# ibrahimhroob/SPS

Hardware: AMD Instinct MI355X
Metric: scans/sec @100k pts, 0.1 m voxel (higher is better)
Workload: dtype f32; 1 GPU; BASELINE config 2: single ~100k-pt LiDAR-like scan + variant-B submap, 0.1 m voxel, CustomMinkUNet14 fp32, 1 scan per step per GPU (4 distinct scans cycled); scan_points=100824, rows=153557, streams_per_gpu=8, compact_arenas=True

## Files before the change

### include/sps_hip.h

```cpp
#ifndef SPS_HIP_H
#define SPS_HIP_H

#include <stddef.h>
#include <stdint.h>

#ifdef __cplusplus
extern "C" {
#endif

#define SPS_OK 0
#define SPS_ERR_INVALID (-1)
#define SPS_ERR_HIP (-2)
#define SPS_ERR_NOMEM (-3)
#define SPS_ERR_RANGE (-4)
#define SPS_ERR_NOWEIGHTS (-5)
#define SPS_ERR_ITEMCAP (-6)

#define SPS_NUM_LEVELS 5

#define SPS_COORD_MIN (-131072)
#define SPS_COORD_MAX (131071)
#define SPS_T_MIN (-16)
#define SPS_T_MAX (15)
#define SPS_BATCH_MAX (30)
#define SPS_MAX_POINTS (1 << 23)

typedef struct sps_ctx sps_ctx;

const char *sps_last_error(void);
int sps_version(void);

int sps_ctx_create(int device, sps_ctx **out);
int sps_ctx_destroy(sps_ctx *ctx);
int sps_reserve(sps_ctx *ctx, int64_t max_points);
int sps_ctx_set_level_fractions(sps_ctx *ctx, const float *frac);
int64_t sps_arena_bytes(sps_ctx *ctx);
int sps_ctx_set_inference_only(sps_ctx *ctx, int on);
int sps_ctx_set_pipelined(sps_ctx *ctx, int on);

int sps_weights_num_tensors(void);
int sps_weights_tensor_info(int idx, char *name, int name_cap, int64_t *offset, int64_t *numel);
int64_t sps_weights_numel(void);
int sps_weights_load(sps_ctx *ctx, const float *blob_host, int64_t numel);
typedef struct sps_weights_handle sps_weights_handle;
int sps_weights_create(int device, const float *blob_host, int64_t numel, int out_channels, sps_weights_handle **out);
int sps_weights_destroy(sps_weights_handle *w);
int sps_ctx_set_weights(sps_ctx *ctx, sps_weights_handle *w);

int sps_forward(sps_ctx *ctx, const float *coords_dev, int64_t ld, int64_t n, float voxel_size,
                float *scores_dev, void *stream);
int sps_check(sps_ctx *ctx, void *stream);

int sps_forward_metrics(sps_ctx *ctx, const float *batch_dev, int64_t ld, int64_t n, float voxel_size, float eps,
                        int n_batches, float *scores_dev, double *out_dev, void *stream);

int sps_head_num_tensors(int out_channels);
int sps_head_tensor_info(int out_channels, int idx, char *name, int name_cap, int64_t *offset, int64_t *numel);
int64_t sps_head_numel(int out_channels);
int sps_weights_load_head(sps_ctx *ctx, const float *blob_host, int64_t numel, int out_channels);
int sps_forward_head(sps_ctx *ctx, const float *coords_dev, int64_t ld, int64_t n, float voxel_size,
                     const float *feats_dev, float t_base, float *out_dev, int64_t ldo, int activation, void *stream);
// ... 206 lines not shown
```

### sps_amd/_native.py

```python
from __future__ import annotations

import ctypes as C
import os

from . import _build

NUM_LEVELS = 5
SPS_OK = 0
ERR_RANGE = -4
ERR_NOMEM = -3
ERR_INVALID = -1
ERR_ITEMCAP = -6


class SpsError(RuntimeError):
    def __init__(self, code: int, msg: str):
        super().__init__(f"libsps_hip error {code}: {msg}")
        self.code = code


ABI_VERSION = 202


def _load() -> C.CDLL:
    path = os.environ.get("SPS_LIB") or _build.LIB
    if path == _build.LIB and (not os.path.exists(path) or _build.is_stale()):
        if _build.have_hipcc():
            path = _build.build()
        elif not os.path.exists(path):
            raise ImportError("libsps_hip.so is missing and hipcc is not available to build it")
    import importlib.util
    if importlib.util.find_spec("torch") is not None:
        import torch
    lib = C.CDLL(path)
    vp, i64, i32, f32 = C.c_void_p, C.c_int64, C.c_int, C.c_float
    sig = {
        "sps_last_error": (C.c_char_p, []),
        "sps_version": (i32, []),
        "sps_ctx_create": (i32, [i32, C.POINTER(vp)]),
        "sps_ctx_destroy": (i32, [vp]),
        "sps_reserve": (i32, [vp, i64]),
        "sps_ctx_set_level_fractions": (i32, [vp, vp]),
        "sps_ctx_set_inference_only": (i32, [vp, i32]),
        "sps_ctx_set_pipelined": (i32, [vp, i32]),
        "sps_arena_bytes": (i64, [vp]),
        "sps_weights_num_tensors": (i32, []),
        "sps_weights_tensor_info": (i32, [i32, C.c_char_p, i32, C.POINTER(i64), C.POINTER(i64)]),
        "sps_weights_numel": (i64, []),
        "sps_weights_load": (i32, [vp, vp, i64]),
        "sps_weights_create": (i32, [i32, vp, i64, i32, C.POINTER(vp)]),
        "sps_weights_destroy": (i32, [vp]),
        "sps_ctx_set_weights": (i32, [vp, vp]),
        "sps_forward": (i32, [vp, vp, i64, i64, f32, vp, vp]),
        "sps_forward_metrics": (i32, [vp, vp, i64, i64, f32, f32, i32, vp, vp, vp]),
        "sps_head_num_tensors": (i32, [i32]),
        "sps_head_tensor_info": (i32, [i32, i32, C.c_char_p, i32, C.POINTER(i64), C.POINTER(i64)]),
        "sps_head_numel": (i64, [i32]),
        "sps_weights_load_head": (i32, [vp, vp, i64, i32]),
        "sps_forward_head": (i32, [vp, vp, i64, i64, f32, vp, f32, vp, i64, i32, vp]),
        "sps_check": (i32, [vp, vp]),
        "sps_metrics": (i32, [vp, vp, vp, i64, i64, f32, i32, C.POINTER(C.c_double), vp]),
        "sps_metrics_dev": (i32, [vp, vp, vp, i64, i64, f32, i32, vp, vp]),
        "sps_profile_enable": (i32, [vp, i32]),
        "sps_profile_count": (i32, [vp]),
        "sps_profile_read": (i32, [vp, i32, C.c_char_p, i32, C.POINTER(f32)]),
        "sps_profile_kernel": (i32, [vp, i32, C.c_char_p, i32]),
        "sps_map_upload": (i32, [vp, vp, i64, i64, f32, vp]),
# ... 81 lines not shown
        "sps_ndt_source_build": (i32, [vp, vp, vp, i64, C.c_double, i32, C.c_double, vp, vp, vp, vp, vp]),
        "sps_ndt_align_d2d_scratch": (i64, [i64]),
        "sps_ndt_align_d2d": (i32, [vp, vp, vp, i64, vp, i32, i32, i32, C.c_double, C.c_double, C.c_double, vp, vp, vp, vp, vp,
                                    vp]),
        "sps_ukf_state_bytes": (i64, []),
        "sps_ukf_init": (i32, [vp, vp, vp, vp, vp]),
        "sps_ukf_predict": (i32, [vp, vp, i32, vp, vp, vp, vp]),
        "sps_ukf_predict_dt": (i32, [vp, C.c_double, vp, vp, vp, vp]),
        "sps_ukf_correct": (i32, [vp, vp, vp, vp, vp, vp]),
    }
    for name, (res, args) in sig.items():
        fn = getattr(lib, name)
        fn.restype = res
        fn.argtypes = args
    if lib.sps_version() != ABI_VERSION:
        raise ImportError(f"{path} reports ABI version {lib.sps_version()}, this binding needs {ABI_VERSION}: rebuild it "
                          "(python -m sps_amd._build)")
    return lib


lib = _load()
EXPORTS = ["sps_last_error", "sps_version", "sps_ctx_create", "sps_ctx_destroy", "sps_reserve",
           "sps_ctx_set_level_fractions", "sps_ctx_set_inference_only", "sps_ctx_set_pipelined", "sps_arena_bytes",
           "sps_weights_num_tensors", "sps_weights_tensor_info", "sps_weights_numel", "sps_weights_load",
           "sps_weights_create", "sps_weights_destroy", "sps_ctx_set_weights",
           "sps_forward", "sps_forward_metrics", "sps_head_num_tensors", "sps_head_tensor_info", "sps_head_numel", "sps_weights_load_head",
           "sps_forward_head", "sps_check", "sps_metrics", "sps_metrics_dev",
           "sps_profile_enable", "sps_profile_count", "sps_profile_read", "sps_profile_kernel", "sps_map_upload", "sps_map_upload_voxels",
           "sps_submap_voxel", "sps_submap_voxel_ijk", "sps_transform_points", "sps_filter_prepare", "sps_forward_n",
           "sps_compact_stable", "sps_filter_finish", "sps_train_forward", "sps_train_backward", "sps_train_generation", "sps_train_backward_at", "sps_scan_mse", "sps_scan_mse_backward", "sps_radius_grid_upload", "sps_radius_count",
           "sps_radius_fill", "sps_radius_grid_attach", "sps_radius_item", "sps_forward_metrics_n", "sps_level_counts", "sps_get_voxels",
           "sps_get_inverse", "sps_get_parent", "sps_get_map_pairs", "sps_get_tile_masks", "sps_get_nbr", "sps_get_kernel_map", "sps_get_rulebook_chunks", "sps_get_logits", "sps_get_feature",
           "sps_lts_num_tensors", "sps_lts_tensor_info", "sps_lts_numel", "sps_lts_lidar_info", "sps_lts_create",
           "sps_lts_destroy", "sps_lts_project", "sps_lts_forward", "sps_lts_check", "sps_lts_tap",
           "sps_forward_head_n", "sps_transform_rows", "sps_transform_points_n", "sps_radius_crop", "sps_label_filter",
           "sps_loc_downsample_scratch", "sps_loc_align_scratch", "sps_loc_downsample", "sps_loc_align",
           "sps_ndt_align_scratch", "sps_ndt_map_build", "sps_ndt_map_cells", "sps_ndt_align",
           "sps_ndt_align_batch_scratch", "sps_ndt_align_batch",
           "sps_ndt_score_scratch", "sps_ndt_score_poses", "sps_ndt_top_poses",
           "sps_ndt_map_build_dynamic", "sps_ndt_map_update_scratch", "sps_ndt_map_update", "sps_ndt_map_info",
           "sps_ndt_map_carve_scratch", "sps_ndt_map_carve", "sps_ndt_map_carve_cells",
           "sps_ndt_pyramid_build", "sps_ndt_pyramid_cells", "sps_ndt_pyramid_align_scratch", "sps_ndt_pyramid_align",
           "sps_ndt_pyramid_build_dynamic", "sps_ndt_pyramid_update_scratch", "sps_ndt_pyramid_update",
           "sps_ndt_pyramid_carve_scratch", "sps_ndt_pyramid_carve", "sps_ndt_pyramid_info", "sps_ndt_pyramid_carve_cells",
           "sps_ndt_source_scratch", "sps_ndt_source_build", "sps_ndt_align_d2d_scratch", "sps_ndt_align_d2d",
           "sps_ukf_state_bytes", "sps_ukf_init", "sps_ukf_predict", "sps_ukf_predict_dt", "sps_ukf_correct"]
# ... 62 lines not shown
            self.handle = None

    def __del__(self):
        try:
            self.close()
        except Exception:
            pass

    def reserve(self, max_points: int):
        check(lib.sps_reserve(self.handle, int(max_points)))

    LIDAR_FRACTIONS = (1.0, 0.6, 0.3, 0.15, 0.08)

    def set_level_fractions(self, frac=None):
        arr = None if frac is None else (C.c_float * NUM_LEVELS)(*[float(x) for x in frac])
        check(lib.sps_ctx_set_level_fractions(self.handle, arr))

    def set_inference_only(self, on: bool = True):
        check(lib.sps_ctx_set_inference_only(self.handle, 1 if on else 0))

    def set_pipelined(self, on: bool = True):
        check(lib.sps_ctx_set_pipelined(self.handle, 1 if on else 0))

    def arena_bytes(self) -> int:
        return int(lib.sps_arena_bytes(self.handle))

    def load_weights(self, blob_host_ptr: int, numel: int, out_channels: int = 1):
        check(lib.sps_weights_load_head(self.handle, blob_host_ptr, int(numel), int(out_channels)))
        self.weights = None

    def set_weights(self, weights: "Weights"):
        check(lib.sps_ctx_set_weights(self.handle, weights.handle))
        self.weights = weights

    def forward_head(self, coords_ptr: int, ld: int, n: int, voxel_size: float, feats_ptr, t_base: float,
                     out_ptr: int, ldo: int, activation: int, stream: int):
        check(lib.sps_forward_head(self.handle, coords_ptr, ld, n, voxel_size, feats_ptr, t_base, out_ptr, ldo,
                                   activation, stream))

    def forward_head_n(self, coords_ptr: int, ld: int, n_max: int, n_dev_ptr: int, voxel_size: float, feats_ptr,
                       t_base: float, out_ptr: int, ldo: int, activation: int, stream: int):
        check(lib.sps_forward_head_n(self.handle, coords_ptr, ld, n_max, n_dev_ptr, voxel_size, feats_ptr, t_base, out_ptr,
                                     ldo, activation, stream))

    def forward_metrics(self, batch_ptr: int, ld: int, n: int, voxel_size: float, eps: float, n_batches: int,
                        scores_ptr: int, out_ptr: int, stream: int):
# ... 364 lines not shown
```

### sps_amd/csrc/grid_kernels.inc.h

```cpp

typedef unsigned int u32x2 __attribute__((ext_vector_type(2)));
constexpr int SCAN_BLOCK = 1024;

struct BHash {
  uint64_t *keys;
  unsigned long long *mask;
  int *first;
  int *rank;
  uint32_t *occ;
  uint32_t hmask;
  uint32_t hshift;
};

constexpr uint32_t BH_X = 0x9E3779B1u, BH_Y = 0x85EBCA77u, BH_Z = 0xC2B2AE3Du, BH_T = 0x27D4EB2Fu;
__device__ inline uint32_t bhash32(uint64_t key) {
  return (uint32_t)(key & 0x3FFFF) * BH_X + (uint32_t)((key >> 18) & 0x3FFFF) * BH_Y + (uint32_t)((key >> 36) & 0x3FFFF) * BH_Z +
         (uint32_t)(key >> 54) * BH_T;
}

__device__ inline int bhash_insert(const BHash &h, uint64_t key) {
  uint32_t s = bhash32(key) >> h.hshift;
  while (true) {
    unsigned long long prev = atomicCAS(reinterpret_cast<unsigned long long *>(&h.keys[s]),
                                        (unsigned long long)KEY_EMPTY, (unsigned long long)key);
// ... 99 lines not shown
}

struct PyramidArgs {
  BHash h[NLV];
  int *sslot[NLV];
  const unsigned char *sbit0;
  int *bslot[NLV];
  uint64_t *bkey[NLV];
  unsigned long long *bmask[NLV];
  int *bbase[NLV];
  uint4 *bmb[NLV];
  int *bparent[NLV];
  int *bchild[NLV];
  int *badj[NLV];
  int *vblock[NLV];
  unsigned char *vbit[NLV];
  int *counts;
  unsigned long long *agg;
  int agg_stride;
  uint32_t gen;
  const int *n_dev;
  int capl[NLV], bcapl[NLV];
  int *err;
};

constexpr int ABORT = 15;

__device__ inline int block_reduce_sum(int v, int *lds) {
  const int lane = threadIdx.x & 63, wave = threadIdx.x >> 6;
  for (int o = 32; o > 0; o >>= 1) v += __shfl_down(v, o, 64);
  if (lane == 0) lds[wave] = v;
  __syncthreads();
  int tot = 0;
  const int nw = blockDim.x >> 6;
  for (int i = 0; i < nw; ++i) tot += lds[i];
  __syncthreads();
  return tot;
}

constexpr int TICKET = 16, TOCC = 24, N_COUNTERS = 32;

__device__ inline unsigned long long agg_pack(uint32_t gen, int t0, int t1) {
  return ((unsigned long long)gen << 32) | ((unsigned long long)(uint32_t)t1 << 13) | (unsigned long long)(uint32_t)t0;
}
constexpr int SCAN_SPIN_MAX = 1 << 22;
__device__ inline int2 scan_lookback(const unsigned long long *agg, int id, uint32_t gen, int *lds, int *err) {
  if constexpr (SPS_ABLATE_FE & 2) return make_int2(0, 0);
// ... 263 lines not shown
          for (int k = 0; k < 2; ++k)
#pragma unroll
            for (int jj = 0; jj < 2; ++jj)
#pragma unroll
              for (int i = 0; i < 2; ++i)
                if (m & (0x0000000000330033ull << (2 * i + 8 * jj + 32 * k))) {
                  const int bit = (int)((2 * oz + k) * 16 + (2 * oy + jj) * 4 + (2 * ox + i));
                  const int row = base + __popcll(pmask & ((1ull << bit) - 1ull));
                  a.vblock[1][row] = br;
                  a.vbit[1][row] = (unsigned char)bit;
                }
        } else {
          const uint32_t px = (bx >> (j - 2)) & 3, py = (by >> (j - 2)) & 3, pz = (bz >> (j - 2)) & 3;
          const int bit = (int)((pz << 4) | (py << 2) | px);
          const int row = base + __popcll(pmask & ((1ull << bit) - 1ull));
          a.vblock[j][row] = br;
          a.vbit[j][row] = (unsigned char)bit;
        }
      }
    }
  }
}

constexpr int LINK_PER = 3;
#if defined(SPS_FE_TRACE)
__device__ unsigned long long g_link_trace[2 * 16384];
struct LinkStamp {
  __device__ LinkStamp() { if (threadIdx.x == 0 && blockIdx.x < 16384) g_link_trace[2 * blockIdx.x] = wall_clock64(); }
  __device__ ~LinkStamp() { if (threadIdx.x == 0 && blockIdx.x < 16384) g_link_trace[2 * blockIdx.x + 1] = wall_clock64(); }
};
#endif
__global__ __launch_bounds__(256) void k_link_adj(PyramidArgs a, int gb, int c1, int c2, int c3, int c4, int c5) {
  if (a.counts[ABORT]) return;
#if defined(SPS_FE_TRACE)
  LinkStamp stamp;
#endif
  if ((int)blockIdx.x < 4 * gb) {
    link_levels(a, (int)blockIdx.x / gb, (int)blockIdx.x % gb, gb);
    return;
  }
  const int bx = (int)blockIdx.x - 4 * gb;
  const int idx = bx < c1 ? 0 : bx < c2 ? 1 : bx < c3 ? 2 : bx < c4 ? 3 : 4;
  const int level = NLV - 1 - idx;
  const int lo = idx == 0 ? 0 : idx == 1 ? c1 : idx == 2 ? c2 : idx == 3 ? c3 : c4;
  const int hi = idx == 0 ? c1 : idx == 1 ? c2 : idx == 2 ? c3 : idx == 3 ? c4 : c5;
  const int total = a.counts[8 + level] * 27;
  const int lim = 1 << (16 - level);
  const BHash h = a.h[level];
  const uint32_t tocc = reinterpret_cast<const uint32_t *>(a.counts)[TOCC];
  const uint64_t *__restrict__ bkey = a.bkey[level];
  int *__restrict__ badj = a.badj[level];
  const __amdgpu_buffer_rsrc_t rsOcc = __builtin_amdgcn_make_buffer_rsrc((void *)h.occ, 0, (int)0xFFFFFFFEu, 0x00020000);
  const __amdgpu_buffer_rsrc_t rsKeys = __builtin_amdgcn_make_buffer_rsrc((void *)h.keys, 0, (int)0xFFFFFFFEu, 0x00020000);
  const __amdgpu_buffer_rsrc_t rsRank = __builtin_amdgcn_make_buffer_rsrc((void *)h.rank, 0, (int)0xFFFFFFFEu, 0x00020000);
  for (int i = (bx - lo) * 256 + (int)threadIdx.x; i < total; i += (hi - lo) * 256) {
    const int r = i / 27, g = i - r * 27;
    const int dy = g % 3 - 1, dz = (g / 3) % 3 - 1, dt = g / 9 - 1;
    const uint64_t key = bkey[r];
    const int kx = (int)(key & 0x3FFFF), ky = (int)((key >> 18) & 0x3FFFF) + dy, kz = (int)((key >> 36) & 0x3FFFF) + dz,
// ... 76 lines not shown
```

### sps_amd/csrc/sps_hip.hip

```cpp
#include <hip/hip_runtime.h>

#include <cmath>
#include <cstdarg>
#include <cstdint>
#include <cstdio>
#include <algorithm>
#include <array>
#include <cstdlib>
#include <cstring>
#include <map>
#include <memory>
#include <string>
#include <vector>

#include "../../include/sps_hip.h"

#if !defined(SPS_DIAG)
#undef SPS_ABLATE_A
#undef SPS_ABLATE_B
#undef SPS_ABLATE_HALF_B
#undef SPS_ABLATE_SKIP_B
#undef SPS_ABLATE_MFMA
#undef SPS_ABLATE_LOOP
#undef SPS_ABLATE_STAGE
// ... 142 lines not shown
  int device = 0;
  float *blob = nullptr;
  float *ss = nullptr;
  float *wu = nullptr;
  float final_bias = 0.f;
  const NetSpec *net = nullptr;
  ~sps_weights() {
    int prev = -1;
    (void)hipGetDevice(&prev);
    (void)hipSetDevice(device);
    (void)hipDeviceSynchronize();
    (void)hipFree(blob);
    (void)hipFree(ss);
    (void)hipFree(wu);
    if (prev >= 0 && prev != device) (void)hipSetDevice(prev);
  }
};
struct sps_weights_handle {
  std::shared_ptr<sps_weights> w;
};

struct sps_train;

struct sps_ctx {
  int device = 0;
  sps_train *train = nullptr;
  int64_t cap = 0;
  int64_t hcap = 0;
  int64_t capl[SPS_NUM_LEVELS] = {}, bcapl[SPS_NUM_LEVELS] = {}, hcapl[SPS_NUM_LEVELS] = {};
  int64_t hash_slots = 0;
  float lfrac[SPS_NUM_LEVELS] = {1.f, 1.f, 1.f, 1.f, 1.f};
  bool compact = false, regrow = false;
  bool lean = false;
  bool pipelined = false;
  uint64_t arena_gen = 0;
  int64_t last_n = 0;
  uint64_t fwd_gen = 0;
  bool have_weights = false;
  std::vector<void *> allocs;
  Level lv[SPS_NUM_LEVELS];
  SubmapScratch sub;
  bool tables_dirty = true;
  void *hash_keys_all = nullptr, *hash_mask_all = nullptr, *hash_first_all = nullptr, *hash_occ_all = nullptr;
  int *nbr5 = nullptr;
  int *counts = nullptr;
  int *err = nullptr;
  int *block_sums = nullptr;
  double *filter_part = nullptr;
  unsigned long long *scan_agg = nullptr;
  int *keep = nullptr;
  double *macc = nullptr;
  unsigned long long *pairs = nullptr;
  std::shared_ptr<sps_weights> weights;
  float *blob = nullptr;
  float *ss = nullptr;
  float *wu = nullptr;
  uint32_t *tm5 = nullptr;
// ... 216 lines not shown
  ALLOC(c->b4t, float, 64 * cl[4]);
  ALLOC(c->b4o, float, 64 * cl[4]);
  c->cap = cap;
  c->hcap = hcap;
  c->last_n = 0;
  ++c->arena_gen;
  HIP_TRY(hipMemset(c->zero_region, 0, zr_words * sizeof(uint32_t)));
  HIP_TRY(hipMemset(c->hash_keys_all, 0xFF, (size_t)hslots * sizeof(uint64_t)));
  HIP_TRY(hipMemset(c->hash_mask_all, 0, (size_t)hslots * sizeof(unsigned long long)));
  HIP_TRY(hipMemset(c->hash_first_all, 0x7F, (size_t)hslots * sizeof(int)));
  HIP_TRY(hipMemset(c->hash_occ_all, 0, (size_t)(hslots / 32) * sizeof(uint32_t)));
  HIP_TRY(hipDeviceSynchronize());
  c->tables_dirty = false;
  return SPS_OK;
}

inline int grid_for(int64_t n, int block, int maxb = 2048) {
  int64_t g = (n + block - 1) / block;
  if (g < 1) g = 1;
  if (g > maxb) g = maxb;
  return (int)g;
}

PyramidArgs pyramid_args(sps_ctx *c) {
  PyramidArgs a{};
  for (int l = 0; l < NLV; ++l) {
    const Level &L = c->lv[l];
    a.h[l] = L.h;
    a.sslot[l] = L.sslot;
    a.bslot[l] = L.bslot;
    a.bkey[l] = L.bkey;
    a.bmask[l] = L.bmask;
    a.bbase[l] = L.bbase;
    a.bmb[l] = L.bmb;
    a.bparent[l] = L.bparent;
    a.bchild[l] = L.bchild;
    a.badj[l] = L.badj;
    a.vblock[l] = L.vblock;
    a.vbit[l] = L.vbit;
  }
  a.counts = c->counts;
  a.sbit0 = c->lv[0].sbit;
  a.agg = c->scan_agg;
  a.agg_stride = (int)(c->cap / SCAN_BLOCK + 8);
  a.gen = (uint32_t)(c->fwd_gen % 0xFFFFFFFFull) + 1u;
  a.n_dev = nullptr;
// ... 17 lines not shown
  float *out;
  int ldo;
  Map map;
  int level_out;
  const float *res;
  int ldr;
  int relu;
  const float *in2 = nullptr;
  int ldi2 = 0;
  bool fin = false;
  const char *up = nullptr;
  float *up_out = nullptr;
  int up_ldo = 0;
};

#ifndef SPS_FUSE_UP
#define SPS_FUSE_UP 12
#endif
constexpr int FUSE_UP = SPS_FUSE_UP;

struct Geometry {
  int ntw, S;
};
Geometry conv_geometry(int level, int K, int cin, int nt, int64_t cap = 0, bool serial_chain = false) {
  if (K == 8 && level >= 3) return {std::min(2, nt), 4};
  if (K == 1 || K == 8) return {nt <= 2 ? nt : 1, 1};
  (void)cin;
  Geometry g = level <= 1 ? Geometry{nt, 1} : Geometry{std::min(2, nt), 4};
  if (serial_chain && K == 81 && level >= 3 && nt >= 2 && cap > 0) {
    const int64_t tiles = std::max<int64_t>(1, cap * (level == 3 ? 33 : 11) / 1000 / 16);
    if (tiles * nt <= 800) g.ntw = 1;
  }
#if defined(SPS_DIAG)
  struct Hook {
    bool set = false;
    int ntw = 1, S = 1;
  };
  static const std::array<Hook, SPS_NUM_LEVELS> hooks = [] {
    std::array<Hook, SPS_NUM_LEVELS> h{};
    for (int l = 0; l < SPS_NUM_LEVELS; ++l) {
      char name[32];
      snprintf(name, sizeof name, "SPS_GEOM_L%d", l);
      const char *e = diag_env(name);
      int ntw = 1, S = 1;
      if (e && sscanf(e, "%d,%d", &ntw, &S) == 2 && (S == 1 || S == 2 || S == 4 || S == 8) && (ntw == 1 || ntw == 2 || ntw == 4))
        h[l] = Hook{true, ntw, S};
    }
    return h;
  }();
  if (level >= 0 && level < SPS_NUM_LEVELS && hooks[level].set) g = {std::min(hooks[level].ntw, nt), hooks[level].S};
#endif
  return g;
}
// ... 64 lines not shown
  ConvArgs a{};
  a.in = cc.in;
  a.ldi = cc.ldi;
  a.out = cc.out;
  a.ldo = cc.ldo;
  a.Wu = c->wu + cs.wu_off;
  a.scale = c->ss + cs.ss_off;
  a.shift = c->ss + cs.ss_off + cs.cout;
  a.res = cc.res;
  a.ldr = cc.ldr;
  a.nbr = cc.map.nbr;
  a.tmask = cc.map.tmask;
  a.ldn = c->capl[cc.level_out];
  a.n_out = c->counts + cc.level_out;
  a.abort_flag = c->counts + 15;
  a.K = cs.K;
  a.cin = cs.cin;
  a.cout = cs.cout;
  a.NT = cs.nt();
  a.upk = cs.upk();
  a.inv_upk = cs.cin >= 4 ? 1.0f / (float)cs.upk() : 1.f;
  a.relu = cc.relu;
  a.in_const = 0.5f;
  const Geometry g = conv_geometry(cc.level_out, cs.K, cs.cin, a.NT, (int64_t)c->cap, !c->pipelined);
  a.S = g.S;
  int64_t gx = (c->cap / 64) >> cc.level_out;
  if (gx < 64) gx = 64;
  if (gx > 4096) gx = 4096;
  {
    static const float gscale = [] { const char *e = diag_env("SPS_GRID_SCALE"); return e ? (float)atof(e) : 1.f; }();
    if (gscale != 1.f) gx = std::max<int64_t>(16, (int64_t)((float)gx * gscale));
  }
  static const int max_wg = [] { const char *e = diag_env("SPS_CONV_MAX_WG"); return e ? atoi(e) : 0; }();
  if (max_wg > 0 && gx * (a.NT / g.ntw) * g.S > max_wg) gx = std::max<int64_t>(16, max_wg / ((a.NT / g.ntw) * g.S));
  dim3 grid((unsigned)(a.NT / g.ntw), (unsigned)(gx * g.S), 1u);
  a.in2 = cc.in2;
  a.ldi2 = cc.ldi2;
  a.upk2 = cs.ds_cin / 4;
  a.in2_bytes = (uint32_t)((size_t)c->capl[cc.level_out] * (size_t)(cc.ldi2 > 0 ? cc.ldi2 : 1) * 4u);
  if (cs.ds_cin > 0 && !cc.in2) return fail(SPS_ERR_INVALID, "%s needs the block input for its fused downsample", cc.name);
  if (cc.fin) {
    const ConvSpec &fs = s.convs[s.find_conv("final")];
    a.fin_w = c->blob + fs.w_off;
    a.fin_b = c->final_bias;
    a.fin_out = c->logits;
  }
  const bool is_up = cs.K == 8 && std::strncmp(cc.name, "convtr", 6) == 0;
  const int level_in = cs.K == 8 ? (is_up ? cc.level_out + 1 : cc.level_out - 1) : cc.level_out;
  a.in_bytes = (uint32_t)((size_t)c->capl[level_in < 0 ? 0 : level_in] * (size_t)cc.ldi * 4u);
  a.wu_bytes = (uint32_t)(cs.wu_numel() * 4);
  a.nbr_bytes = (uint32_t)((size_t)cs.K * (size_t)c->capl[cc.level_out] * 4u);
// ... 3 lines not shown
  if (cc.up) {
    const ConvSpec &us = s.convs[s.find_conv(cc.up)];
    if (us.cin != cs.cout || cc.level_out < 1) return fail(SPS_ERR_INVALID, "%s cannot be fused into %s", cc.up, cc.name);
    a.up_Wu = c->wu + us.wu_off;
    a.up_scale = c->ss + us.ss_off;
    a.up_shift = c->ss + us.ss_off + us.cout;
    a.up_down = c->lv[cc.level_out].down;
    a.up_tmask = c->lv[cc.level_out].tmdown;
    a.up_ldn = c->capl[cc.level_out];
    a.up_out = cc.up_out;
    a.up_ldo = cc.up_ldo;
    a.up_cout = us.cout;
    a.up_rows = (int)c->capl[cc.level_out - 1];
    a.up_wu_bytes = (uint32_t)(us.wu_numel() * 4);
    grid.x = 1;
    a.order_ways = TILE_ORDER == 2 ? TILE_ORDER_WAYS : 0;
  }
  {
    static const char *trace_layer = diag_env("SPS_TRACE_LAYER");
    a.trace_on = trace_layer && std::strcmp(trace_layer, cc.name) == 0;
  }
  if (cs.cin == 1) {
    TileOrderArgs to{};
    const int g0 = grid_for(c->cap, 64, 4096);
    int gto = 0;
    if (TILE_ORDER != 0) {
      for (int l = 0; l < NLV; ++l) {
        const bool px = l < PX_LEVELS && ((px_levels() >> l) & 1) && c->lv[l].px_order;
        to.tm3[l] = (c->lv[l].nbr3 || !px) ? c->lv[l].tm3 : nullptr, to.order[l] = c->lv[l].tile_order;
        to.rb_cnt[l] = px ? c->lv[l].rb_cnt : nullptr, to.px_sorted[l] = c->lv[l].px_sorted, to.px_order[l] = c->lv[l].px_order;
      }
      to.counts = c->counts;
      gto = NLV - TILE_ORDER_FIRST_LEVEL + PX_LEVELS;
    }
    c->last_kernel = c->cur_vfeat ? "k_conv0_feat" : "k_conv0_fused";
    {
      static const int c0mode = [] { const char *e = diag_env("SPS_DIAG_CONV0"); return e ? atoi(e) : 0; }();
      if (c0mode == 1) {
        hipLaunchKernelGGL(k_conv0_fused, dim3((unsigned)gto), dim3(256), 0, st, a.n_out, c->lv[0].view(), c->blob + cs.w_off, a.scale,
                           a.shift, a.in_const, a.out, a.ldo, 1, to, 0);
        return SPS_OK;
      }
      if (c0mode == 2) gto = 0;
    }
    if (c->cur_vfeat) {
      hipLaunchKernelGGL(k_conv0_feat, dim3((unsigned)(g0 + gto)), dim3(256), 0, st, a.n_out,
                         c->lv[0].view(), c->blob + cs.w_off, a.scale, a.shift, c->cur_vfeat, a.out, a.ldo, to, g0);
      return SPS_OK;
    }
    hipLaunchKernelGGL(k_conv0_fused, dim3((unsigned)(g0 + gto)), dim3(256), 0, st, a.n_out,
                       c->lv[0].view(), c->blob + cs.w_off, a.scale, a.shift, a.in_const, a.out, a.ldo, 1, to, g0);
    return SPS_OK;
  }
  if (cs.K == 8 && std::strncmp(cc.name, "convtr", 6) == 0) {
    {
      const int coarse = cc.level_out + 1;
      a.nbr = c->lv[coarse].down;
      a.tmask = c->lv[coarse].tmdown;
      a.n_out = c->counts + coarse;
      a.ldn = c->capl[coarse];
      a.tile_cap = (int)(c->capl[coarse] / 16);
      a.out_rows = (int)c->capl[cc.level_out];
      int64_t gu = (c->cap / 16) >> coarse;
      if (gu < 64) gu = 64;
      if (gu > 8192) gu = 8192;
      const dim3 gr((unsigned)gu);
      c->last_kernel = "k_upconv";
      if (a.NT == 1)
        hipLaunchKernelGGL((k_upconv<1>), gr, dim3(256), 0, st, a);
      else if (a.NT == 2)
        hipLaunchKernelGGL((k_upconv<2>), gr, dim3(256), 0, st, a);
      else
        hipLaunchKernelGGL((k_upconv<4>), gr, dim3(256), 0, st, a);
      return SPS_OK;
    }
  }
  const bool ds = cs.ds_cin > 0;
  if (cc.level_out < PX_LEVELS && ((px_levels() >> cc.level_out) & 1) && c->lv[cc.level_out].rb_e && cs.K == 81 && a.NT == 1 && (cs.cout == 8 || cs.cout == 16) &&
      (cs.cin == 8 || cs.cin == 16 || cs.cin == 24) && (!cc.fin || cs.cout == 8)) {
    int64_t gs = (c->cap / 64) >> cc.level_out;
    if (gs < 64) gs = 64;
    if (gs > 4096) gs = 4096;
    const dim3 gridp((unsigned)gs);
    a.rb_e = c->lv[cc.level_out].rb_e;
    a.rb_k = c->lv[cc.level_out].rb_k;
    a.rb_cnt = c->lv[cc.level_out].rb_cnt;
    a.px_order = TILE_ORDER != 0 ? c->lv[cc.level_out].px_order : nullptr;
    a.rb_supertiles = (int)(c->capl[cc.level_out] / 64);
    const int key = cs.cin * 100 + (cs.cout == 8 ? 10 : 0) + (cc.fin ? 2 : (ds ? 1 : 0));
    c->last_kernel = "k_conv_px";
    static_assert(PX_HALF_LEVELS == 1, "SPS_PX_LAUNCH picks the HALF instantiations for level 0 alone");
    if (px_half_level(cc.level_out) && cs.cout != 8)
      return fail(SPS_ERR_INVALID, "%s: C_out = %d cannot read the 8-pair rulebook of level %d", cc.name, cs.cout, cc.level_out);
#define SPS_PX_LAUNCH(CIN_, C8_, DS_, FIN_)                                                                  \
  do {                                                                                                       \
    if (cc.level_out == 0)                                                                                   \
      launch_px<SPS_PX0, CIN_, C8_, DS_, FIN_, SPS_PX0_W, false, C8_>(gridp, st, a);                         \
    else                                                                                                     \
      launch_px<SPS_PX1, CIN_, C8_, DS_, FIN_, SPS_PX1_W>(gridp, st, a);                                     \
  } while (0)
    switch (key) {
      case 800: SPS_PX_LAUNCH(8, false, false, false); break;
      case 810: SPS_PX_LAUNCH(8, true, false, false); break;
      case 811: SPS_PX_LAUNCH(8, true, true, false); break;
      case 812: SPS_PX_LAUNCH(8, true, true, true); break;
// ... 118 lines not shown
  return SPS_OK;
}

}

extern "C" {

const char *sps_last_error(void) { return g_err.c_str(); }
int sps_version(void) { return 202; }

int sps_ctx_create(int device, sps_ctx **out) {
  if (!out) return fail(SPS_ERR_INVALID, "out is null");
  int ndev = 0;
  HIP_TRY(hipGetDeviceCount(&ndev));
  if (device < 0 || device >= ndev) return fail(SPS_ERR_INVALID, "device %d out of range (%d devices)", device, ndev);
  HIP_TRY(hipSetDevice(device));
  sps_ctx *c = new sps_ctx();
  c->device = device;
  c->net = &spec(1);
  HIP_TRY(hipMalloc((void **)&c->err, sizeof(int)));
  HIP_TRY(hipMalloc((void **)&c->macc, 32 * 8 * sizeof(double)));
  HIP_TRY(hipMalloc((void **)&c->pairs, 128 * sizeof(unsigned long long)));
  HIP_TRY(hipMemset(c->err, 0, sizeof(int)));
  *out = c;
  return SPS_OK;
}

static void train_destroy(sps_ctx *c);

int sps_ctx_destroy(sps_ctx *c) {
  if (!c) return SPS_OK;
  (void)hipSetDevice(c->device);
  (void)hipDeviceSynchronize();
  train_destroy(c);
  free_arena(c);
  (void)hipFree(c->err);
  (void)hipFree(c->macc);
  (void)hipFree(c->pairs);
  c->weights.reset();
  if (c->map_keys_alloc) (void)hipFree(c->map_keys_alloc);
  for (void *p : c->rg_allocs) (void)hipFree(p);
  for (void *p : c->ndt_allocs) (void)hipFree(p);
  for (void *p : c->ndt_pyr_allocs) (void)hipFree(p);
  for (void *p : {(void *)c->item_counts, (void *)c->item_offsets, (void *)c->item_bsum, (void *)c->item_base}) (void)hipFree(p);
  delete c;
  return SPS_OK;
}

int sps_reserve(sps_ctx *c, int64_t max_points) {
  if (!c || max_points < 0) return fail(SPS_ERR_INVALID, "bad arguments");
  if (max_points > SPS_MAX_POINTS) return fail(SPS_ERR_INVALID, "max_points too large (limit %d)", SPS_MAX_POINTS);
  return reserve(c, max_points < 1024 ? 1024 : max_points);
}

int sps_weights_num_tensors(void) { return (int)spec().tensors.size(); }

int sps_weights_tensor_info(int idx, char *name, int name_cap, int64_t *offset, int64_t *numel) {
  const NetSpec &s = spec();
  if (idx < 0 || idx >= (int)s.tensors.size()) return fail(SPS_ERR_INVALID, "tensor index %d out of range", idx);
  const TensorInfo &t = s.tensors[idx];
  if (name && name_cap > 0) {
// ... 224 lines not shown
  if (!c) return fail(SPS_ERR_INVALID, "ctx is null");
  if (!c->have_weights) return fail(SPS_ERR_NOWEIGHTS, "sps_weights_load has not been called");
  if (n < 0 || ld < 5 || (n > 0 && (!coords || !scores))) return fail(SPS_ERR_INVALID, "bad arguments");
  if (!(vs > 0.f)) return fail(SPS_ERR_INVALID, "voxel_size must be > 0");
  if (n > SPS_MAX_POINTS) return fail(SPS_ERR_INVALID, "too many points (limit %d)", SPS_MAX_POINTS);
  HIP_TRY(hipSetDevice(c->device));
  hipStream_t st = (hipStream_t)stream;
  if (n > c->cap || c->regrow) {
    int rc = reserve(c, n);
    if (rc != SPS_OK) return rc;
  }
  static const int diag_skip = [] { const char *e = diag_env("SPS_DIAG_SKIP"); return e ? atoi(e) : 0; }();
  static const int no_merge = [] { const char *e = diag_env("SPS_NO_MERGE"); return e ? atoi(e) : 0; }();
  const bool skip_front = (diag_skip & 1) && c->last_n == n && c->diag_have_state;
  const bool skip_convs = (diag_skip & 2) != 0;
  c->last_n = n;
  ++c->fwd_gen;
  const int64_t cap = c->cap;
  c->prof_n = 0;
  prof_mark(c, "begin", st);
  Level &L0 = c->lv[0];
  PyramidArgs pa = pyramid_args(c);
  pa.n_dev = fo.n_dev;
  if (!skip_front) {
  if (c->tables_dirty) {
    HIP_TRY(hipMemsetAsync(c->hash_keys_all, 0xFF, (size_t)c->hash_slots * sizeof(uint64_t), st));
    HIP_TRY(hipMemsetAsync(c->hash_mask_all, 0, (size_t)c->hash_slots * sizeof(unsigned long long), st));
    HIP_TRY(hipMemsetAsync(c->hash_first_all, 0x7F, (size_t)c->hash_slots * sizeof(int), st));
    HIP_TRY(hipMemsetAsync(c->hash_occ_all, 0, (size_t)(c->hash_slots / 32) * sizeof(uint32_t), st));
  }
  if (c->tables_dirty) HIP_TRY(hipMemsetAsync(c->zero_region, 0, c->zero_bytes, st));
  c->tables_dirty = true;
  if (n == 0) {
    HIP_TRY(hipMemsetAsync(c->zero_region, 0, c->zero_bytes, st));
    c->tables_dirty = false;
    return SPS_OK;
  }
  prof_mark(c, "reset", st);

  const unsigned gp = (unsigned)((n + 255) / 256);
  const unsigned gs0 = (unsigned)((n + SCAN_BLOCK - 1) / SCAN_BLOCK);
  const unsigned gsb = (unsigned)((cap + SCAN_BLOCK * RANK_ITEMS - 1) / (SCAN_BLOCK * RANK_ITEMS));
  hipLaunchKernelGGL(k_points_to_blocks, dim3(gp), dim3(256), 0, st, coords, ld, (int)n, vs, fo.t_base, L0.h, L0.sslot, L0.sbit,
                     c->err, reinterpret_cast<uint4 *>(c->zero_region), (int)(c->zero_bytes / 16), fo.metrics_out,
                     fo.metrics_out ? fo.n_batches * 8 : 0, fo.n_dev);
  hipLaunchKernelGGL(k_rank_points, dim3(gs0), dim3(SCAN_BLOCK), 0, st, pa, (int)n);
  hipLaunchKernelGGL(k_rank_blocks_rows, dim3(4 * gsb + gs0), dim3(SCAN_BLOCK), 0, st, pa, (int)gsb, (int)n, L0.inv);
  const int gb = grid_for(cap >> 2, 256, 256);
  if (fo.feats) {
    HIP_TRY(hipMemsetAsync(c->vacc, 0, (size_t)n * sizeof(long long), st));
    HIP_TRY(hipMemsetAsync(c->vcnt, 0, (size_t)n * sizeof(int), st));
    hipLaunchKernelGGL(k_voxel_feat_accum, dim3(gp), dim3(256), 0, st, fo.feats, L0.inv, (int)n, c->vacc, c->vcnt, fo.n_dev);
    hipLaunchKernelGGL(k_voxel_feat_mean, dim3((unsigned)grid_for(n, 256, 2048)), dim3(256), 0, st, c->counts, c->vacc,
                       c->vcnt, c->vfeat);
  }
  c->last_kernel = "k_points_to_blocks+k_rank_points+k_rank_blocks_rows";
  prof_mark(c, "voxelize", st);
  {
    int co[NLV + 1] = {0};
    for (int i = 0; i < NLV; ++i) co[i + 1] = co[i] + grid_for(((cap >> 3) >> (2 * (NLV - 1 - i))) * 27, 256, 2048);
#if defined(SPS_FE_TRACE)
    g_link_geom[0] = gb;
    for (int l = 0; l <= NLV; ++l) g_link_geom[1 + l] = co[l];
#endif
    if (no_merge & 2) {
      hipLaunchKernelGGL(k_link_adj, dim3(4 * gb), dim3(256), 0, st, pa, gb, co[1], co[2], co[3], co[4], co[5]);
      hipLaunchKernelGGL(k_link_adj, dim3(co[NLV]), dim3(256), 0, st, pa, 0, co[1], co[2], co[3], co[4], co[5]);
    } else {
      hipLaunchKernelGGL(k_link_adj, dim3(4 * gb + co[NLV]), dim3(256), 0, st, pa, gb, co[1], co[2], co[3], co[4], co[5]);
    }
  }
  c->last_kernel = "k_link_adj";
  prof_mark(c, "pyramid", st);
  MapsArgs ma{};
  int off = 0;
  for (int l = 0; l < NLV; ++l) {
    const Level &L = c->lv[l];
    ma.L[l] = L.view();
    ma.nbr3[l] = L.nbr3;
    ma.tm3[l] = L.tm3;
    ma.down[l] = L.down;
    ma.parent_row[l] = L.inv;
    ma.tmdown[l] = L.tmdown;
    ma.chunk_off[l] = off;
    off += grid_for(cap >> l, 256, 1024);
  }
  ma.chunk_off[NLV] = off;
  ma.counts = c->counts;
  for (int l = 0; l < PX_LEVELS; ++l)
    if (((px_levels() >> l) & 1) && !fo.front_only) ma.rb_e[l] = c->lv[l].rb_e, ma.rb_k[l] = c->lv[l].rb_k, ma.rb_cnt[l] = c->lv[l].rb_cnt;
  for (int l = 0; l < NLV; ++l) ma.ldn[l] = c->capl[l];
#if defined(SPS_FE_TRACE)
  g_maps_geom[0] = off;
  for (int l = 0; l <= NLV; ++l) g_maps_geom[1 + l] = ma.chunk_off[l];
#endif
  if (no_merge & 4) {
    hipLaunchKernelGGL(k_maps, dim3(off * 3), dim3(256), 0, st, ma, off, off * 3);
    hipLaunchKernelGGL(k_maps, dim3(ma.chunk_off[NLV - 1]), dim3(256), 0, st, ma, off, 0);
  } else {
    hipLaunchKernelGGL(k_maps, dim3(off * 3 + ma.chunk_off[NLV - 1]), dim3(256), 0, st, ma, off, off * 3);
  }
  c->diag_have_state = true;
  }
  c->last_kernel = "k_maps";
  prof_mark(c, "maps", st);
  if (fo.front_only) {
    HIP_TRY(hipGetLastError());
    return SPS_OK;
// ... 41 lines not shown
  for (const ConvCall &cc : calls) {
    if (skip_convs) break;
    if (skip_class) {
      const bool tr = std::strncmp(cc.name, "convtr", 6) == 0, c0 = std::strcmp(cc.name, "conv0p1s1") == 0;
      const bool blk = std::strncmp(cc.name, "block", 5) == 0, strided = !tr && !c0 && !blk;
      const int cls = blk ? (cc.level_out >= 2 ? 1 : 2) : strided ? 4 : tr ? 8 : 16;
      if (skip_class & cls) continue;
    }
    if (fused_up && std::strcmp(cc.name, fused_up) == 0) {
      fused_up = nullptr;
      continue;
    }
    int rc = run_conv(c, cc, st);
    if (rc != SPS_OK) return rc;
    const char *stage = cc.name;
    if (cc.up) {
      fused_up = cc.up;
      for (const auto &fs : fused_stage)
        if (std::strcmp(cc.name, fs[0]) == 0) stage = fs[1];
    }
    prof_mark(c, stage, st);
  }
  c->cur_vfeat = nullptr;
  const int gs = (int)((n + 255) / 256), gbc = grid_for(cap >> 2, 256, 256);
  if (fo.head) {
    const NetSpec &s = *c->net;
    const ConvSpec &fs = s.convs[s.find_conv("final")];
    hipLaunchKernelGGL(k_slice_head, dim3((unsigned)gs), dim3(256), 0, st, c->b8o, 8, L0.inv, (int)n,
                       c->blob + fs.w_off, c->blob + s.bias_off, s.out_channels, fo.act, scores, fo.ldo, c->counts + 15,
                       fo.n_dev);
    c->last_kernel = "k_slice_head";
    prof_mark(c, "slice_head", st);
    if (!skip_front) hipLaunchKernelGGL(k_bhash_cleanup, dim3(gbc * NLV), dim3(256), 0, st, pa, gbc);
  } else if (skip_front || (no_merge & 8)) {
    hipLaunchKernelGGL(k_slice_sigmoid, dim3((unsigned)gs), dim3(256), 0, st, c->logits, L0.inv, (int)n, scores, c->counts + 15);
    if (!skip_front) hipLaunchKernelGGL(k_bhash_cleanup, dim3(gbc * NLV), dim3(256), 0, st, pa, gbc);
    if (fo.metrics_out) {
      HIP_TRY(hipMemsetAsync(fo.metrics_out, 0, (size_t)fo.n_batches * 8 * sizeof(double), st));
      hipLaunchKernelGGL(k_metrics, dim3((unsigned)grid_for(n, 1024, 128)), dim3(256), 0, st, scores, (int)n,
                         MetricsArgs{coords, ld, fo.eps, fo.n_batches, fo.metrics_out});
    }
  } else {
    const MetricsArgs mt{coords, ld, fo.eps, fo.n_batches, fo.metrics_out};
    const int gst = fo.metrics_out ? grid_for(n, 1024, 256) : gs;
    hipLaunchKernelGGL(k_tail, dim3((unsigned)(gst + gbc * NLV)), dim3(256), 0, st, c->logits, L0.inv, (int)n, scores, gst,
                       pa, gbc, mt);
  }
// ... 725 lines not shown
```

Baseline: 4109 scans/s.

## Size kernel grids from device-posted row counts via mapped-host mailbox

The pyramid link kernel now writes each level's observed row and block counts, plus the point count and a generation number, into a mapped pinned-host mailbox. On the next forward the host reads the last two observations, scales them to the current point count with a 25% margin, and uses the result to size grids for voxelize, link, maps, conv, upconv and cleanup kernels. It also feeds the conv tile geometry heuristic. Previously these grids were sized from arena capacity, so the aim is to stop launching blocks that would sit idle. This depends on the kernels handling more rows than the launched grid covers, for example through grid-stride loops. It also adds a host read of device-written memory and an API to pin the hint manually.

```diff
diff --git a/include/sps_hip.h b/include/sps_hip.h
--- a/include/sps_hip.h
+++ b/include/sps_hip.h
@@ -37,6 +37,10 @@
 int64_t sps_arena_bytes(sps_ctx *ctx);
 int sps_ctx_set_inference_only(sps_ctx *ctx, int on);
 int sps_ctx_set_pipelined(sps_ctx *ctx, int on);
+int sps_ctx_set_grid_hint(sps_ctx *ctx, const int32_t rows[6]);
+int sps_ctx_get_grid_hint(sps_ctx *ctx, int32_t rows[6], int64_t *n_rows, uint32_t *generation);
+int64_t sps_grid_hint_rows(int64_t cap_rows, int64_t count_a, int64_t n_a, int64_t count_b, int64_t n_b, int64_t n_now);
+int sps_grid_hint_blocks(int64_t cap_rows, int64_t hint_rows, int rows_per_block, int floor_blocks, int max_blocks);
 
 int sps_weights_num_tensors(void);
 int sps_weights_tensor_info(int idx, char *name, int name_cap, int64_t *offset, int64_t *numel);
diff --git a/sps_amd/_native.py b/sps_amd/_native.py
--- a/sps_amd/_native.py
+++ b/sps_amd/_native.py
@@ -43,6 +43,10 @@
         "sps_ctx_set_level_fractions": (i32, [vp, vp]),
         "sps_ctx_set_inference_only": (i32, [vp, i32]),
         "sps_ctx_set_pipelined": (i32, [vp, i32]),
+        "sps_ctx_set_grid_hint": (i32, [vp, C.POINTER(C.c_int32)]),
+        "sps_ctx_get_grid_hint": (i32, [vp, C.POINTER(C.c_int32), C.POINTER(i64), C.POINTER(C.c_uint32)]),
+        "sps_grid_hint_rows": (i64, [i64, i64, i64, i64, i64, i64]),
+        "sps_grid_hint_blocks": (i32, [i64, i64, i32, i32, i32]),
         "sps_arena_bytes": (i64, [vp]),
         "sps_weights_num_tensors": (i32, []),
         "sps_weights_tensor_info": (i32, [i32, C.c_char_p, i32, C.POINTER(i64), C.POINTER(i64)]),
@@ -170,6 +174,7 @@
 lib = _load()
 EXPORTS = ["sps_last_error", "sps_version", "sps_ctx_create", "sps_ctx_destroy", "sps_reserve",
            "sps_ctx_set_level_fractions", "sps_ctx_set_inference_only", "sps_ctx_set_pipelined", "sps_arena_bytes",
+           "sps_ctx_set_grid_hint", "sps_ctx_get_grid_hint", "sps_grid_hint_rows", "sps_grid_hint_blocks",
            "sps_weights_num_tensors", "sps_weights_tensor_info", "sps_weights_numel", "sps_weights_load",
            "sps_weights_create", "sps_weights_destroy", "sps_ctx_set_weights",
            "sps_forward", "sps_forward_metrics", "sps_head_num_tensors", "sps_head_tensor_info", "sps_head_numel", "sps_weights_load_head",
@@ -278,6 +283,15 @@
     def set_pipelined(self, on: bool = True):
         check(lib.sps_ctx_set_pipelined(self.handle, 1 if on else 0))
 
+    def set_grid_hint(self, rows=None):
+        arr = None if rows is None else (C.c_int32 * 6)(*[int(x) for x in rows])
+        check(lib.sps_ctx_set_grid_hint(self.handle, arr))
+
+    def grid_hint(self):
+        rows, n, gen = (C.c_int32 * 6)(), C.c_int64(0), C.c_uint32(0)
+        check(lib.sps_ctx_get_grid_hint(self.handle, rows, C.byref(n), C.byref(gen)))
+        return list(rows), int(n.value), int(gen.value)
+
     def arena_bytes(self) -> int:
         return int(lib.sps_arena_bytes(self.handle))
 
diff --git a/sps_amd/csrc/grid_kernels.inc.h b/sps_amd/csrc/grid_kernels.inc.h
--- a/sps_amd/csrc/grid_kernels.inc.h
+++ b/sps_amd/csrc/grid_kernels.inc.h
@@ -145,7 +145,16 @@
   const int *n_dev;
   int capl[NLV], bcapl[NLV];
   int *err;
+  int *mail;
+  int mail_n;
 };
+
+constexpr int MAIL_ROWS = 0;
+constexpr int MAIL_BLOCKS0 = 5;
+constexpr int MAIL_N = 6;
+constexpr int MAIL_GEN = 7;
+constexpr int MAIL_BLOCKS1 = 8;
+constexpr int MAIL_WORDS = 16;
 
 constexpr int ABORT = 15;
 
@@ -455,6 +464,23 @@
   }
 }
 
+typedef int i32x4 __attribute__((ext_vector_type(4)));
+__device__ inline void mailbox_post(const PyramidArgs &a) {
+  if (!a.mail) return;
+  const int *np = a.n_dev ? a.n_dev : a.counts;
+  int rows[NLV], blocks[NLV];
+#pragma unroll
+  for (int l = 0; l < NLV; ++l) rows[l] = a.counts[l], blocks[l] = a.counts[8 + l];
+  const int nd = *np;
+  const int n = a.n_dev ? min(a.mail_n, nd) : a.mail_n;
+  if (n <= 0) return;
+  static_assert(NLV == 5 && MAIL_ROWS == 0 && MAIL_BLOCKS0 == 5 && MAIL_N == 6 && MAIL_GEN == 7 && MAIL_BLOCKS1 == 8, "mailbox layout");
+  volatile i32x4 *m = reinterpret_cast<volatile i32x4 *>(a.mail);
+  m[0] = i32x4{rows[0], rows[1], rows[2], rows[3]};
+  m[2] = i32x4{blocks[1], blocks[2], blocks[3], blocks[4]};
+  m[1] = i32x4{rows[4], blocks[0], n, (int)a.gen};
+}
+
 constexpr int LINK_PER = 3;
 #if defined(SPS_FE_TRACE)
 __device__ unsigned long long g_link_trace[2 * 16384];
@@ -468,6 +494,7 @@
 #if defined(SPS_FE_TRACE)
   LinkStamp stamp;
 #endif
+  if (blockIdx.x == gridDim.x - 1 && threadIdx.x == 0) mailbox_post(a);
   if ((int)blockIdx.x < 4 * gb) {
     link_levels(a, (int)blockIdx.x / gb, (int)blockIdx.x % gb, gb);
     return;
diff --git a/sps_amd/csrc/sps_hip.hip b/sps_amd/csrc/sps_hip.hip
--- a/sps_amd/csrc/sps_hip.hip
+++ b/sps_amd/csrc/sps_hip.hip
@@ -188,6 +188,16 @@
 
 struct sps_train;
 
+struct GridObs {
+  uint32_t gen = 0;
+  int64_t n = 0;
+  int64_t rows[SPS_NUM_LEVELS] = {}, blocks[SPS_NUM_LEVELS] = {};
+};
+struct GridHint {
+  int64_t rows[SPS_NUM_LEVELS] = {}, blocks[SPS_NUM_LEVELS] = {};
+  int64_t expect[SPS_NUM_LEVELS] = {};
+};
+
 struct sps_ctx {
   int device = 0;
   sps_train *train = nullptr;
@@ -199,6 +209,12 @@
   bool compact = false, regrow = false;
   bool lean = false;
   bool pipelined = false;
+  int32_t *mail = nullptr;
+  int *mail_dev = nullptr;
+  GridObs obs[2];
+  bool hint_pinned = false;
+  int32_t pin[6] = {};
+  GridHint gh;
   uint64_t arena_gen = 0;
   int64_t last_n = 0;
   uint64_t fwd_gen = 0;
@@ -461,6 +477,62 @@
   return (int)g;
 }
 
+int64_t hint_rows_of(int64_t cap_rows, int64_t count_a, int64_t n_a, int64_t count_b, int64_t n_b, int64_t n_now, int margin_pct) {
+  int64_t best = -1;
+  const int64_t cnt[2] = {count_a, count_b}, nn[2] = {n_a, n_b};
+  for (int i = 0; i < 2; ++i) {
+    if (nn[i] <= 0 || cnt[i] < 0) continue;
+    const int64_t den = 100 * nn[i];
+    const int64_t v = (cnt[i] * std::max<int64_t>(n_now, 0) * (100 + margin_pct) + den - 1) / den;
+    best = std::max(best, v);
+  }
+  if (best < 0) return 0;
+  return std::min(std::max<int64_t>(best, 1), std::max<int64_t>(cap_rows, 1));
+}
+
+int hint_blocks_of(int64_t cap_rows, int64_t hint_rows, int rows_per_block, int floor_blocks, int max_blocks) {
+  const int64_t rpb = std::max(rows_per_block, 1), lo = std::max(floor_blocks, 1), hi = std::max<int64_t>(max_blocks, lo);
+  const int64_t g_cap = std::min(std::max((std::max<int64_t>(cap_rows, 0) + rpb - 1) / rpb, lo), hi);
+  if (hint_rows <= 0) return (int)g_cap;
+  return (int)std::min(std::max((hint_rows + rpb - 1) / rpb, lo), g_cap);
+}
+
+constexpr int GRID_HINT_MARGIN_PCT = 25;
+
+void grid_hint_poll(sps_ctx *c) {
+  if (!c->mail) return;
+  const volatile int32_t *m = c->mail;
+  GridObs o;
+  o.gen = (uint32_t)m[MAIL_GEN];
+  if (o.gen == 0) return;
+  o.n = m[MAIL_N];
+  for (int l = 0; l < NLV; ++l) o.rows[l] = m[MAIL_ROWS + l];
+  o.blocks[0] = m[MAIL_BLOCKS0];
+  for (int l = 1; l < NLV; ++l) o.blocks[l] = m[MAIL_BLOCKS1 + l - 1];
+  if (o.n <= 0) return;
+  if (o.gen != c->obs[0].gen) c->obs[1] = c->obs[0];
+  c->obs[0] = o;
+}
+
+GridHint grid_hint_for(sps_ctx *c, int64_t n_now) {
+  GridHint h;
+  if (c->hint_pinned) {
+    for (int l = 0; l < NLV; ++l) {
+      h.rows[l] = h.expect[l] = std::max<int64_t>(1, c->pin[l]);
+      h.blocks[l] = std::max<int64_t>(1, (int64_t)c->pin[5] >> (2 * l));
+    }
+    return h;
+  }
+  grid_hint_poll(c);
+  const GridObs &a = c->obs[0], &b = c->obs[1];
+  for (int l = 0; l < NLV; ++l) {
+    h.rows[l] = hint_rows_of(c->capl[l], a.rows[l], a.n, b.rows[l], b.n, n_now, GRID_HINT_MARGIN_PCT);
+    h.expect[l] = hint_rows_of(c->capl[l], a.rows[l], a.n, b.rows[l], b.n, n_now, 0);
+    h.blocks[l] = hint_rows_of(c->bcapl[l], a.blocks[l], a.n, b.blocks[l], b.n, n_now, GRID_HINT_MARGIN_PCT);
+  }
+  return h;
+}
+
 PyramidArgs pyramid_args(sps_ctx *c) {
   PyramidArgs a{};
   for (int l = 0; l < NLV; ++l) {
@@ -524,13 +596,13 @@
 struct Geometry {
   int ntw, S;
 };
-Geometry conv_geometry(int level, int K, int cin, int nt, int64_t cap = 0, bool serial_chain = false) {
+Geometry conv_geometry(int level, int K, int cin, int nt, int64_t cap = 0, bool serial_chain = false, int64_t expect_rows = 0) {
   if (K == 8 && level >= 3) return {std::min(2, nt), 4};
   if (K == 1 || K == 8) return {nt <= 2 ? nt : 1, 1};
   (void)cin;
   Geometry g = level <= 1 ? Geometry{nt, 1} : Geometry{std::min(2, nt), 4};
   if (serial_chain && K == 81 && level >= 3 && nt >= 2 && cap > 0) {
-    const int64_t tiles = std::max<int64_t>(1, cap * (level == 3 ? 33 : 11) / 1000 / 16);
+    const int64_t tiles = expect_rows > 0 ? (expect_rows + 15) / 16 : std::max<int64_t>(1, cap * (level == 3 ? 33 : 11) / 1000 / 16);
     if (tiles * nt <= 800) g.ntw = 1;
   }
 #if defined(SPS_DIAG)
@@ -641,11 +713,10 @@
   a.inv_upk = cs.cin >= 4 ? 1.0f / (float)cs.upk() : 1.f;
   a.relu = cc.relu;
   a.in_const = 0.5f;
-  const Geometry g = conv_geometry(cc.level_out, cs.K, cs.cin, a.NT, (int64_t)c->cap, !c->pipelined);
+  const GridHint &gh = c->gh;
+  const Geometry g = conv_geometry(cc.level_out, cs.K, cs.cin, a.NT, (int64_t)c->cap, !c->pipelined, gh.expect[cc.level_out]);
   a.S = g.S;
-  int64_t gx = (c->cap / 64) >> cc.level_out;
-  if (gx < 64) gx = 64;
-  if (gx > 4096) gx = 4096;
+  int64_t gx = hint_blocks_of(c->cap >> cc.level_out, gh.rows[cc.level_out], 64, 64, 4096);
   {
     static const float gscale = [] { const char *e = diag_env("SPS_GRID_SCALE"); return e ? (float)atof(e) : 1.f; }();
     if (gscale != 1.f) gx = std::max<int64_t>(16, (int64_t)((float)gx * gscale));
@@ -695,7 +766,7 @@
   }
   if (cs.cin == 1) {
     TileOrderArgs to{};
-    const int g0 = grid_for(c->cap, 64, 4096);
+    const int g0 = hint_blocks_of(c->cap, gh.rows[0], 64, 1, 4096);
     int gto = 0;
     if (TILE_ORDER != 0) {
       for (int l = 0; l < NLV; ++l) {
@@ -734,9 +805,7 @@
       a.ldn = c->capl[coarse];
       a.tile_cap = (int)(c->capl[coarse] / 16);
       a.out_rows = (int)c->capl[cc.level_out];
-      int64_t gu = (c->cap / 16) >> coarse;
-      if (gu < 64) gu = 64;
-      if (gu > 8192) gu = 8192;
+      const int gu = hint_blocks_of(c->cap >> coarse, gh.rows[coarse], 16, 64, 8192);
       const dim3 gr((unsigned)gu);
       c->last_kernel = "k_upconv";
       if (a.NT == 1)
@@ -751,9 +820,7 @@
   const bool ds = cs.ds_cin > 0;
   if (cc.level_out < PX_LEVELS && ((px_levels() >> cc.level_out) & 1) && c->lv[cc.level_out].rb_e && cs.K == 81 && a.NT == 1 && (cs.cout == 8 || cs.cout == 16) &&
       (cs.cin == 8 || cs.cin == 16 || cs.cin == 24) && (!cc.fin || cs.cout == 8)) {
-    int64_t gs = (c->cap / 64) >> cc.level_out;
-    if (gs < 64) gs = 64;
-    if (gs > 4096) gs = 4096;
+    const int gs = hint_blocks_of(c->cap >> cc.level_out, gh.rows[cc.level_out], 64, 64, 4096);
     const dim3 gridp((unsigned)gs);
     a.rb_e = c->lv[cc.level_out].rb_e;
     a.rb_k = c->lv[cc.level_out].rb_k;
@@ -918,7 +985,42 @@
   HIP_TRY(hipMalloc((void **)&c->macc, 32 * 8 * sizeof(double)));
   HIP_TRY(hipMalloc((void **)&c->pairs, 128 * sizeof(unsigned long long)));
   HIP_TRY(hipMemset(c->err, 0, sizeof(int)));
+  HIP_TRY(hipHostMalloc((void **)&c->mail, MAIL_WORDS * sizeof(int32_t), hipHostMallocMapped));
+  std::memset(c->mail, 0, MAIL_WORDS * sizeof(int32_t));
+  HIP_TRY(hipHostGetDevicePointer((void **)&c->mail_dev, c->mail, 0));
   *out = c;
+  return SPS_OK;
+}
+
+int64_t sps_grid_hint_rows(int64_t cap_rows, int64_t count_a, int64_t n_a, int64_t count_b, int64_t n_b, int64_t n_now) {
+  return hint_rows_of(cap_rows, count_a, n_a, count_b, n_b, n_now, GRID_HINT_MARGIN_PCT);
+}
+
+int sps_grid_hint_blocks(int64_t cap_rows, int64_t hint_rows, int rows_per_block, int floor_blocks, int max_blocks) {
+  return hint_blocks_of(cap_rows, hint_rows, rows_per_block, floor_blocks, max_blocks);
+}
+
+int sps_ctx_set_grid_hint(sps_ctx *c, const int32_t rows[6]) {
+  if (!c) return fail(SPS_ERR_INVALID, "ctx is null");
+  c->hint_pinned = rows != nullptr;
+  for (int i = 0; i < 6; ++i) c->pin[i] = rows ? rows[i] : 0;
+  return SPS_OK;
+}
+
+int sps_ctx_get_grid_hint(sps_ctx *c, int32_t rows[6], int64_t *n_rows, uint32_t *generation) {
+  if (!c || !rows) return fail(SPS_ERR_INVALID, "null argument");
+  if (c->hint_pinned) {
+    for (int i = 0; i < 6; ++i) rows[i] = c->pin[i];
+    if (n_rows) *n_rows = 0;
+    if (generation) *generation = 0;
+    return SPS_OK;
+  }
+  grid_hint_poll(c);
+  const GridObs &o = c->obs[0];
+  for (int l = 0; l < NLV; ++l) rows[l] = (int32_t)o.rows[l];
+  rows[5] = (int32_t)o.blocks[0];
+  if (n_rows) *n_rows = o.n;
+  if (generation) *generation = o.gen;
   return SPS_OK;
 }
 
@@ -933,6 +1035,7 @@
   (void)hipFree(c->err);
   (void)hipFree(c->macc);
   (void)hipFree(c->pairs);
+  if (c->mail) (void)hipHostFree(c->mail);
   c->weights.reset();
   if (c->map_keys_alloc) (void)hipFree(c->map_keys_alloc);
   for (void *p : c->rg_allocs) (void)hipFree(p);
@@ -1203,6 +1306,9 @@
   Level &L0 = c->lv[0];
   PyramidArgs pa = pyramid_args(c);
   pa.n_dev = fo.n_dev;
+  c->gh = n > 0 ? grid_hint_for(c, n) : GridHint{};
+  const GridHint &gh = c->gh;
+  pa.mail = c->mail_dev, pa.mail_n = (int)n;
   if (!skip_front) {
   if (c->tables_dirty) {
     HIP_TRY(hipMemsetAsync(c->hash_keys_all, 0xFF, (size_t)c->hash_slots * sizeof(uint64_t), st));
@@ -1227,7 +1333,7 @@
                      fo.metrics_out ? fo.n_batches * 8 : 0, fo.n_dev);
   hipLaunchKernelGGL(k_rank_points, dim3(gs0), dim3(SCAN_BLOCK), 0, st, pa, (int)n);
   hipLaunchKernelGGL(k_rank_blocks_rows, dim3(4 * gsb + gs0), dim3(SCAN_BLOCK), 0, st, pa, (int)gsb, (int)n, L0.inv);
-  const int gb = grid_for(cap >> 2, 256, 256);
+  const int gb = hint_blocks_of(cap >> 2, gh.blocks[0], 256, 1, 256);
   if (fo.feats) {
     HIP_TRY(hipMemsetAsync(c->vacc, 0, (size_t)n * sizeof(long long), st));
     HIP_TRY(hipMemsetAsync(c->vcnt, 0, (size_t)n * sizeof(int), st));
@@ -1239,7 +1345,10 @@
   prof_mark(c, "voxelize", st);
   {
     int co[NLV + 1] = {0};
-    for (int i = 0; i < NLV; ++i) co[i + 1] = co[i] + grid_for(((cap >> 3) >> (2 * (NLV - 1 - i))) * 27, 256, 2048);
+    for (int i = 0; i < NLV; ++i) {
+      const int l = NLV - 1 - i;
+      co[i + 1] = co[i] + hint_blocks_of(((cap >> 3) >> (2 * l)) * 27, gh.blocks[l] * 27, 256, 1, 2048);
+    }
 #if defined(SPS_FE_TRACE)
     g_link_geom[0] = gb;
     for (int l = 0; l <= NLV; ++l) g_link_geom[1 + l] = co[l];
@@ -1264,7 +1373,7 @@
     ma.parent_row[l] = L.inv;
     ma.tmdown[l] = L.tmdown;
     ma.chunk_off[l] = off;
-    off += grid_for(cap >> l, 256, 1024);
+    off += hint_blocks_of(cap >> l, gh.rows[l], 256, 1, 1024);
   }
   ma.chunk_off[NLV] = off;
   ma.counts = c->counts;
@@ -1352,7 +1461,7 @@
     prof_mark(c, stage, st);
   }
   c->cur_vfeat = nullptr;
-  const int gs = (int)((n + 255) / 256), gbc = grid_for(cap >> 2, 256, 256);
+  const int gs = (int)((n + 255) / 256), gbc = hint_blocks_of(cap >> 2, gh.blocks[0], 256, 1, 256);
   if (fo.head) {
     const NetSpec &s = *c->net;
     const ConvSpec &fs = s.convs[s.find_conv("final")];
```

Result: no change. 4159 scans/s (median of 6 runs) (+1.2%).
